# smellslikeml/distributed-deep-learning-workshop

Hardware: AMD Instinct MI355X
Metric: images/sec (whole node) ResNet-50 224px (higher is better)
Workload: dtype bf16; 1 GPU; model=resnet50, global_batch=256, per_gpu_batch=256, image_size=224, parallelism=dp1, hip_ops=True, conv_routes=hip

## Files before the change

ddlw_amd/ops/abi.py:

```python
from __future__ import annotations

import ctypes
from ctypes import POINTER, c_char_p, c_float, c_int, c_long, c_ulonglong


class Ptr(ctypes.c_void_p):

    @classmethod
    def from_param(cls, v):
        if v is None or isinstance(v, int):
            return ctypes.c_void_p(v)
        return ctypes.c_void_p(v.data_ptr())


def long_array(values):
    return (c_long * len(values))(*values)


def int_array(values):
    return (c_int * len(values))(*values)


_P, _I, _L, _F = Ptr, c_int, c_long, c_float

SIGNATURES = {
    "ddlw_last_error": (c_char_p, []),
    "ddlw_device_sync": (_I, []),
    "ddlw_bn_nparts": (_I, [_L, _I]),
    "ddlw_bn_stats": (_I, [_P, _P, _P, _L, _I, _P]),
    "ddlw_bn_parts_fold": (_I, [_P, _P, _P, _P, _L, _I, _I, _P]),
    "ddlw_bn_finalize": (_I, [_P] * 6 + [_L, _I, _I, _F, _F, _P]),
    "ddlw_bn_apply": (_I, [_P] * 8 + [_L, _I, _I, _P]),
    "ddlw_bn_bwd_reduce": (_I, [_P] * 7 + [_L, _I, _I, _P]),
    "ddlw_bn_grad_finalize": (_I, [_P, _P, _P, _P, _I, _I, _P]),
    "ddlw_bn_bwd_dx": (_I, [_P] * 10 + [_L, _I, _I, _P]),
    "ddlw_maxpool3x3s2_fwd": (_I, [_P, _P, _P] + [_I] * 6 + [_P]),
    "ddlw_maxpool3x3s2_bwd": (_I, [_P, _P, _P] + [_I] * 6 + [_P]),
    "ddlw_gap_fwd": (_I, [_P, _P, _I, _I, _I, _P]),
    "ddlw_gap_bwd": (_I, [_P, _P, _I, _I, _I, _P]),
    "ddlw_softmax_ce": (_I, [_P, _P, _P, _P, _I, _I, _F, _P]),
    "ddlw_dropout_fwd": (_I, [_P, _P, _P, _L, _F, c_ulonglong, _P]),
    "ddlw_dropout_bwd": (_I, [_P, _P, _P, _L, _F, _P]),
    "ddlw_argmax_rows": (_I, [_P, _P, _L, _I, _P]),
    "ddlw_accuracy": (_I, [_P, _P, _P, _L, _I, _P]),
    "ddlw_ce_metrics_nblocks": (_I, [_I, _I, _P]),
    "ddlw_ce_metrics": (_I, [_P] * 6 + [_I, _I, _F, _I, _P]),
    "ddlw_normalize_u8": (_I, [_P, _P, _L, _P]),
    "ddlw_fused_sgd": (_I, [_P, _I, _L, _F, _F, _F, _I, _P]),
    "ddlw_fused_adam": (_I, [_P, _I, _L, _F, _F, _F, _F, _F, _F, _F, _P]),
    "ddlw_fused_adadelta": (_I, [_P, _I, _L, _F, _F, _F, _F, _P]),
    "ddlw_depthwise_fwd": (_I, [_P, _P, _P] + [_I] * 10 + [_P]),
    "ddlw_depthwise_fwd_ep": (_I, [_P] * 5 + [_I] * 9 + [_P]),
    "ddlw_depthwise_dgrad": (_I, [_P, _P, _P] + [_I] * 10 + [_P]),
    "ddlw_depthwise_wgrad_nparts": (_I, [_L, _I]),
    "ddlw_depthwise_wgrad": (_I, [_P, _P, _P, _P] + [_I] * 10 + [_P]),
    "ddlw_pw_conv_fwd": (_I, [_P] * 6 + [_I, _L, _I, _I, _P]),
    "ddlw_pw_conv_nparts": (_I, [_L, _I, _P]),
    "ddlw_pw_conv_fwd_stats": (_I, [_P] * 5 + [_L, _I, _I, _P]),
    "ddlw_conv_fwd_nparts": (_L, [_I] * 8),
    "ddlw_conv_fwd_igemm": (_I, [_P] * 14 + [_I] * 15 + [_P]),
    "ddlw_conv_dgrad_s2m": (_I, [_P] * 4 + [_I] * 9
                            + [POINTER(c_long), POINTER(c_long), POINTER(c_int), _P]),
    "ddlw_conv_wgrad": (_I, [_P] * 5 + [_I] * 12 + [_P]),
    "ddlw_stem_repack": (_I, [_P, _P, _I, _I, _I, _P]),
    "ddlw_conv_stem": (_I, [_P] * 4 + [_I] * 8 + [_P, _P, _I, _P]),
    "ddlw_stem_wgrad": (_I, [_P] * 5 + [_I] * 7 + [_P]),
    "ddlw_stem3_u8_fwd_ep": (_I, [_P] * 5 + [_I] * 6 + [_P]),
}


def apply(cdll, on_missing) -> None:
    for name, (restype, argtypes) in SIGNATURES.items():
        try:
            fn = getattr(cdll, name)
        except AttributeError:
            on_missing(name)
            raise
        fn.restype = restype
        fn.argtypes = argtypes
```

ddlw_amd/ops/conv_gemm.py:

```python
from __future__ import annotations

import json
import os
from pathlib import Path
from typing import Tuple

import torch

from .abi import int_array, long_array
from .runtime import launch, query

_DISPATCH_PATH = Path(__file__).resolve().parent / "conv_dispatch.json"
_dispatch = None


def _table() -> dict:
    global _dispatch
    if _dispatch is None:
        if _DISPATCH_PATH.exists():
            _dispatch = json.loads(_DISPATCH_PATH.read_text())
        else:
            _dispatch = {}
    return _dispatch


def _key(N, H, W, C, K, R, S, stride) -> str:
    return f"{N}x{H}x{W}x{C}-{K}k{R}x{S}s{stride}"


def fwd_supported(C: int, K: int, R: int, S: int) -> bool:
    return C % 64 == 0


def dgrad_supported(C: int, K: int, stride, R: int = 1, pad: int = 0) -> bool:
    s = stride[0] if isinstance(stride, (tuple, list)) else stride
    if K % 64 != 0:
        return False
    if s == 1:
        return True
    return s == 2 and ((R == 1 and pad == 0) or (R == 3 and pad == 1))


_zpage = {}


def _zero_page(device) -> torch.Tensor:
    t = _zpage.get(device)
    if t is None:
        t = torch.zeros(64, dtype=torch.bfloat16, device=device)
        _zpage[device] = t
    return t


def _route(kind: str, shape_key: str, mode: str, supported: bool) -> bool:
    if not supported:
        return False
    if mode == "hip":
        return True
    if mode == "stock":
        return False
    ent = _table().get(shape_key)
    if ent is None:
        return False
    return ent.get(kind, "stock") == "hip"


def _pair(v) -> Tuple[int, int]:
    return (v, v) if isinstance(v, int) else (int(v[0]), int(v[1]))


def _igemm(x, w, y, N, H, W, C, K, Ho, Wo, R, S, stride, pad, oH, oW, oS,
           acc=None, parts=None, bnb=(None,) * 4, ep=(None, None, 0),
           acc_mask=None):
    ps, pq = (None, None) if parts is None else (parts[0], parts[1])
    launch("conv_fwd_igemm", x, w, y, _zero_page(x.device), acc, acc_mask,
           ps, pq, *bnb,
           ep[0], ep[1], 1 if ep[2] else 0,
           N, H, W, C, K, Ho, Wo, R, S, stride, pad, oH, oW, oS)


def conv_fwd_kernel(x: torch.Tensor, weight: torch.Tensor, stride, padding,
                    acc: torch.Tensor = None, bn_parts: bool = False,
                    bnb=None, ep=None, acc_mask: torch.Tensor = None):
    n, c, h, w = x.shape
    k, _, r, s = weight.shape
    st, _ = _pair(stride)
    pd, _ = _pair(padding)
    ho = (h + 2 * pd - r) // st + 1
    wo = (w + 2 * pd - s) // st + 1
    x = x.contiguous(memory_format=torch.channels_last)
    weight = weight.contiguous(memory_format=torch.channels_last)
    y = torch.empty((n, k, ho, wo), dtype=torch.bfloat16, device=x.device,
                    memory_format=torch.channels_last)
    if acc is not None:
        assert acc.shape == y.shape and acc.dtype == torch.bfloat16
        acc = acc.contiguous(memory_format=torch.channels_last)
    if acc_mask is not None and acc is not None:
        assert (acc_mask.dtype == torch.uint8 and acc_mask.is_contiguous()
                and acc_mask.numel() * 8 == y.numel())
    bnb_args, ep_args = (None,) * 4, (None, None, 0)
    parts = np_ = None
    if ep is not None:
        ep_args = ep
    elif bnb is not None or bn_parts:
        if bnb is not None:
            bx, bmask, bmean, brstd = bnb
            bx = bx.contiguous(memory_format=torch.channels_last)
            bnb_args = (bx, bmask, bmean, brstd)
        else:
            assert acc is None
        np_ = int(query("conv_fwd_nparts", n, c, k, ho, wo, r, s,
                        1 if bnb is not None else 0))
        parts = torch.empty(2, np_, k, dtype=torch.float32, device=x.device)
    _igemm(x, weight, y, n, h, w, c, k, ho, wo, r, s, st, pd, ho, wo, 1,
           acc, parts, bnb_args, ep_args, acc_mask)
    return y if parts is None else (y, parts, np_)


def wgrad_supported(C: int, K: int) -> bool:
    return C % 8 == 0 and K % 8 == 0


def _wgrad_split(M: int, K: int, C: int, RS: int) -> int:
    bk = 128 if K >= 128 else 64
    bc = 128 if C >= 128 else 64
    base = ((K + bk - 1) // bk) * ((C + bc - 1) // bc) * RS
    split = max(1, min(1024 // max(base, 1), 1024, M // 64 or 1))
    return split


def conv_wgrad_kernel(dy: torch.Tensor, x: torch.Tensor, weight_shape,
                      stride, padding) -> torch.Tensor:
    n, c, h, w = x.shape
    k, _, r, s = weight_shape
    st, _ = _pair(stride)
    pd, _ = _pair(padding)
    ho, wo = dy.shape[2], dy.shape[3]
    M = n * ho * wo
    split = _wgrad_split(M, k, c, r * s)
    x = x.contiguous(memory_format=torch.channels_last)
    dy = dy.contiguous(memory_format=torch.channels_last)
    elems = k * r * s * c
    slab = torch.empty(split * elems, dtype=torch.float32, device=x.device)
    dw = torch.empty((k, c, r, s), dtype=torch.bfloat16, device=x.device,
                     memory_format=torch.channels_last)
    launch("conv_wgrad", dy, x, _zero_page(x.device), slab, dw,
           n, h, w, c, k, ho, wo, r, s, st, pd, split)
    return dw


def conv_dgrad_kernel(dy: torch.Tensor, weight: torch.Tensor, in_shape,
                      padding, stride=1, acc: torch.Tensor = None, bnb=None,
                      acc_mask: torch.Tensor = None):
    k, c, r, s = weight.shape
    pd, _ = _pair(padding)
    st, _ = _pair(stride)
    wt = weight.flip(2, 3).permute(1, 0, 2, 3)
    wt = wt.contiguous(memory_format=torch.channels_last)
    if st == 1:
        return conv_fwd_kernel(dy, wt, 1, r - 1 - pd, acc=acc, bnb=bnb,
                               acc_mask=acc_mask)
    assert acc is None and acc_mask is None, \
        "fused accumulate: stride-1 dgrad only"
    assert bnb is None, "fused BN-bwd reduce: stride-1 dgrad only"
    if st == 2 and r == 3 and pd == 1:
        return _conv_dgrad_s2_3x3(dy, weight, in_shape)
    assert st == 2 and r == 1 and pd == 0, "scatter dgrad: 1x1 s2 pad0 only"
    n, _, ho, wo = dy.shape
    _, _, ih, iw = in_shape
    dy = dy.contiguous(memory_format=torch.channels_last)
    dx = torch.empty((n, c, ih, iw), dtype=torch.bfloat16, device=dy.device,
                     memory_format=torch.channels_last).zero_()
    _igemm(dy, wt, dx, n, ho, wo, k, c, ho, wo, 1, 1, 1, 0, ih, iw, 2)
    return dx


def _raw_fwd_scatter(x, wflat, y_ptr, N, H, W, C, K, Ho, Wo, R, S,
                     oH, oW, oS):
    _igemm(x, wflat, y_ptr, N, H, W, C, K, Ho, Wo, R, S, 1, 0, oH, oW, oS)


def _conv_dgrad_s2_3x3(dy: torch.Tensor, weight: torch.Tensor, in_shape) -> torch.Tensor:
    k, c, _, _ = weight.shape
    n, _, ih, iw = in_shape
    ho, wo = dy.shape[2], dy.shape[3]
    dy = dy.contiguous(memory_format=torch.channels_last)
    dx = torch.empty((n, c, ih, iw), dtype=torch.bfloat16, device=dy.device,
                     memory_format=torch.channels_last)
    classes = []
    for dh in (0, 1):
        taps_r = [r for r in (2, 1, 0) if (dh + 1 - r) % 2 == 0]
        for dw_ in (0, 1):
            taps_s = [t for t in (2, 1, 0) if (dw_ + 1 - t) % 2 == 0]
            sub = weight[:, :, taps_r][:, :, :, taps_s]
            wf = sub.permute(1, 0, 2, 3).contiguous(
                memory_format=torch.channels_last)
            classes.append((dh, dw_, len(taps_r), len(taps_s),
                            (dh * iw + dw_) * c, wf))
    if ih % 2 == 0 and iw % 2 == 0 and k % 64 == 0:
        wcat = torch.cat([wf.permute(0, 2, 3, 1).reshape(-1)
                          for *_, wf in classes])
        woffs = [0]
        for *_, wf in classes[:-1]:
            woffs.append(woffs[-1] + wf.numel())
        launch("conv_dgrad_s2m", dy, wcat, dx, _zero_page(dy.device),
               n, ho, wo, k, c, ih // 2, iw // 2, ih, iw,
               long_array(woffs),
               long_array([off for _, _, _, _, off, _ in classes]),
               int_array([v for _, _, nr, ns, _, _ in classes for v in (nr, ns)]))
        return dx
    for dh, dw_, nr, ns, off_elems, wf in classes:
        oh = (ih - dh + 1) // 2
        ow = (iw - dw_ + 1) // 2
        _raw_fwd_scatter(
            dy, wf, dx.data_ptr() + off_elems * dx.element_size(),
            n, ho, wo, k, c, oh, ow, nr, ns, ih, iw, 2,
        )
    return dx


def conv_backward(dy, x, weight, stride, padding, hip_dgrad, hip_wgrad,
                  need_dx=True, need_dw=True, acc=None, acc_mask=None):
    if acc_mask is not None and not (need_dx and hip_dgrad
                                     and _pair(stride)[0] == 1):
        raise ValueError("conv_backward: acc_mask needs the stride-1 HIP dgrad")
    dy = dy.contiguous(memory_format=torch.channels_last)
    if dy.is_cuda and dy.dtype != torch.bfloat16:
        dy = dy.to(torch.bfloat16)
    st, _ = _pair(stride)
    dx = dw = None
    if need_dx and hip_dgrad:
        fuse = acc if st == 1 else None
        dx = conv_dgrad_kernel(dy, weight.to(torch.bfloat16), x.shape,
                               padding, stride, acc=fuse, acc_mask=acc_mask)
        if acc is not None and fuse is None:
            dx = dx + acc
    if need_dw and hip_wgrad:
        dw = conv_wgrad_kernel(dy, x, weight.shape, stride, padding)
        if dw.dtype != weight.dtype:
            dw = dw.to(weight.dtype)
    if (need_dw and dw is None) or (need_dx and dx is None):
        mask_dx = bool(need_dx and dx is None)
        mask_dw = bool(need_dw and dw is None)
        w16 = weight.to(dy.dtype)
        gi, gw, _ = torch.ops.aten.convolution_backward(
            dy, x, w16, None,
            list(stride) if isinstance(stride, (tuple, list)) else [stride] * 2,
            list(padding) if isinstance(padding, (tuple, list)) else [padding] * 2,
            [1, 1], False, [0, 0], 1,
            [mask_dx, mask_dw, False],
        )
        if mask_dx:
            dx = gi if acc is None else gi + acc
        if mask_dw:
            dw = gw.to(weight.dtype)
    return dx, dw


class _ConvFn(torch.autograd.Function):
    @staticmethod
    def forward(ctx, x, weight, bias, stride, padding, hip_fwd, hip_dgrad,
                hip_wgrad):
        ctx.save_for_backward(x, weight)
        ctx.stride, ctx.padding = stride, padding
        ctx.hip_dgrad = hip_dgrad
        ctx.hip_wgrad = hip_wgrad
        ctx.has_bias = bias is not None
        if hip_fwd:
            y = conv_fwd_kernel(x, weight.to(torch.bfloat16), stride, padding)
        else:
            y = torch.nn.functional.conv2d(
                x, weight.to(x.dtype), None, stride, padding
            )
        if bias is not None:
            y = y + bias.to(y.dtype).view(1, -1, 1, 1)
        return y

    @staticmethod
    def backward(ctx, dy):
        x, weight = ctx.saved_tensors
        dx, dw = conv_backward(
            dy, x, weight, ctx.stride, ctx.padding,
            ctx.hip_dgrad, ctx.hip_wgrad,
            need_dx=ctx.needs_input_grad[0], need_dw=ctx.needs_input_grad[1],
        )
        db = None
        if ctx.has_bias and ctx.needs_input_grad[2]:
            db = dy.float().sum(dim=(0, 2, 3))
        return dx, dw, db, None, None, None, None, None


def available(mod, x: torch.Tensor, mode: str) -> bool:
    if mode == "stock":
        return False
    cache = getattr(mod, "_ddlw_cache", None)
    sig = (tuple(x.shape), mode)
    if cache is not None and cache[0] == sig:
        mod._ddlw_route = cache[1]
        return cache[1][0] or cache[1][1]
    n, c, h, w = x.shape
    k, _, r, s = mod.weight.shape
    st, _ = _pair(mod.stride)
    key = _key(n, h, w, c, k, r, s, st)
    pd0 = mod.padding[0] if isinstance(mod.padding, (tuple, list)) else mod.padding
    f = _route("fwd", key, mode, fwd_supported(c, k, r, s))
    d = _route("dgrad", key, mode, dgrad_supported(c, k, mod.stride, r, pd0))
    g = _route("wgrad", key, mode, wgrad_supported(c, k))
    mod._ddlw_route = (f, d, g)
    mod._ddlw_cache = (sig, (f, d, g))
    return f or d or g


def conv2d(x, weight, bias, stride, padding, hip_fwd: bool, hip_dgrad: bool,
           hip_wgrad: bool = False):
    return _ConvFn.apply(x, weight, bias, stride, padding, hip_fwd, hip_dgrad,
                         hip_wgrad)




def _stem_repack(x: torch.Tensor) -> torch.Tensor:
    n, _, h, w = x.shape
    x4 = torch.empty((n, h, w + 8, 4), dtype=torch.bfloat16, device=x.device)
    launch("stem_repack", x, x4, n, h, w)
    return x4


def stem_fwd_kernel(x: torch.Tensor, weight: torch.Tensor,
                    ep=None) -> torch.Tensor:
    n, c, h, w = x.shape
    k = weight.shape[0]
    assert c == 3 and k == 64 and weight.shape[2:] == (7, 7)
    ho, wo = (h + 6 - 7) // 2 + 1, (w + 6 - 7) // 2 + 1
    x = x.contiguous(memory_format=torch.channels_last)
    dev = x.device
    x4 = _stem_repack(x)
    w4 = torch.zeros(k, 8, 8, 4, dtype=torch.bfloat16, device=dev)
    w4[:, :7, :7, :3] = weight.detach().to(torch.bfloat16).permute(0, 2, 3, 1)
    y = torch.empty((n, k, ho, wo), dtype=torch.bfloat16, device=dev,
                    memory_format=torch.channels_last)
    es, eb, relu = ep if ep is not None else (None, None, False)
    launch("conv_stem", x4, w4, y, _zero_page(dev), n, h, w, k, ho, wo, 2, 3,
           es, eb, 1 if relu else 0)
    return y


def stem_wgrad_kernel(dy: torch.Tensor, x: torch.Tensor) -> torch.Tensor:
    n, c, h, w = x.shape
    assert c == 3
    ho, wo = dy.shape[2], dy.shape[3]
    x = x.contiguous(memory_format=torch.channels_last)
    dy = dy.contiguous(memory_format=torch.channels_last)
    dev = x.device
    x4 = _stem_repack(x)
    split = int(min(1024, max(1, (n * ho * wo) // 64)))
    slab = torch.empty(split * 64 * 256, dtype=torch.float32, device=dev)
    dw4 = torch.empty(64, 256, dtype=torch.bfloat16, device=dev)
    launch("stem_wgrad", dy, x4, _zero_page(dev), slab, dw4,
           n, h, w, 64, ho, wo, split)
    dw = (dw4.view(64, 8, 8, 4)[:, :7, :7, :3]
          .permute(0, 3, 1, 2)
          .contiguous(memory_format=torch.channels_last))
    return dw


class _StemFn(torch.autograd.Function):
    @staticmethod
    def forward(ctx, x, weight):
        ctx.save_for_backward(x, weight)
        return stem_fwd_kernel(x, weight)

    @staticmethod
    def backward(ctx, dy):
        x, weight = ctx.saved_tensors
        dy = dy.contiguous(memory_format=torch.channels_last)
        dx = dw = None
        if ctx.needs_input_grad[0]:
            dx = torch.nn.grad.conv2d_input(
                list(x.shape), weight.to(dy.dtype), dy, (2, 2), (3, 3))
        if ctx.needs_input_grad[1]:
            if dy.is_cuda and dy.dtype == torch.bfloat16:
                dw = stem_wgrad_kernel(dy, x).to(weight.dtype)
            else:
                dw = torch.nn.grad.conv2d_weight(
                    x.to(dy.dtype), list(weight.shape), dy, (2, 2), (3, 3))
        return dx, dw


def stem_conv2d(x: torch.Tensor, weight: torch.Tensor) -> torch.Tensor:
    return _StemFn.apply(x, weight)
```

ddlw_amd/ops/hip/conv_wgrad.hip:

```cpp
#include "igemm.h"

typedef __attribute__((ext_vector_type(8))) __bf16 bf16x8_v;
typedef __attribute__((ext_vector_type(4))) float f32x4_v;
typedef __attribute__((ext_vector_type(2))) unsigned tr64_t;

__device__ __forceinline__ unsigned lds_u32(const bf16_t* p) {
  return (unsigned)(unsigned long long)(const LDS_AS bf16_t*)p;
}

template <int BK, int BC, int WG_BM = 64>
__global__ __launch_bounds__(256) void k_conv_wgrad(
    const bf16_t* __restrict__ dy, const bf16_t* __restrict__ x,
    const bf16_t* __restrict__ zpage,
    float* __restrict__ slab,
    int N, int H, int W_, int C, int K, int Ho, int Wo,
    int R, int S, int stride, int pad,
    int split, long m_per_split,
    unsigned long long magic_wo, unsigned shift_wo,
    unsigned long long magic_ho, unsigned shift_ho) {
  constexpr int WK = BK / 2, WC = BC / 2;
  constexpr int KF = WK / 16, CF = WC / 16;
  constexpr int MG = WG_BM / 32;
  constexpr int PA = BK / 16 * MG;
  constexpr int PB = BC / 16 * MG;
  constexpr int TILE = WG_BM * BK;
  constexpr int BUF = WG_BM * (BK + BC);
  __shared__ __attribute__((aligned(16))) bf16_t smem[2 * BUF];

  const long M = (long)N * Ho * Wo;
  const int ctiles = (C + BC - 1) / BC;
  const int tile_k = blockIdx.x / ctiles;
  const int tile_c = blockIdx.x % ctiles;
  const int rs = blockIdx.y;
  const int r = rs / S, s = rs % S;
  const int sp = blockIdx.z;

  const long m0 = (long)sp * m_per_split;
  const long m1 = (m0 + m_per_split < M) ? (m0 + m_per_split) : M;

  const int tid = threadIdx.x;
  const int lane = tid & 63;
  const int wave = tid >> 6;
  const int wr = wave >> 1, wc2 = wave & 1;

  const int s_pos = lane >> 3;
  const int s_mr = (lane >> 1) & 3;
  const int s_half = lane & 1;
  const int s_mb = (s_pos < 4) ? (2 * s_pos) : (2 * (s_pos - 4) + 1);
  const int s_mlocal = s_mb * 4 + s_mr;
  const int s_koff = s_half * 8;

  const bf16_t* dyrow[MG];
  const bf16_t* xrow[MG];
  bool dv[MG], xv[MG];

  auto decompose = [&](long mbase) {
    #pragma unroll
    for (int g = 0; g < MG; ++g) {
      long m = mbase + g * 32 + s_mlocal;
      dv[g] = m < m1;
      dyrow[g] = dv[g] ? (dy + m * K) : zpage;
      bool ok = false;
      const bf16_t* xr = zpage;
      if (m < m1) {
        unsigned mu = (unsigned)m;
        unsigned q1 = mdiv(mu, magic_wo, shift_wo);
        int wo = (int)(mu - q1 * (unsigned)Wo);
        unsigned n_u = mdiv(q1, magic_ho, shift_ho);
        int ho = (int)(q1 - n_u * (unsigned)Ho);
        int hh = ho * stride - pad + r;
        int wwv = wo * stride - pad + s;
        ok = hh >= 0 && hh < H && wwv >= 0 && wwv < W_;
        if (ok) xr = x + (((long)(int)n_u * H + hh) * W_ + wwv) * C;
      }
      xv[g] = ok;
      xrow[g] = xr;
    }
  };

  auto stage = [&](int buf) {
    bf16_t* ldy = smem + buf * BUF;
    bf16_t* lx = ldy + TILE;
    #pragma unroll
    for (int p = wave; p < PA; p += 4) {
      const int k16 = p / MG, g = p % MG;
      int kk = tile_k * BK + k16 * 16 + s_koff;
      const bf16_t* src = (dv[g] && kk < K) ? (dyrow[g] + kk) : zpage;
      __builtin_amdgcn_global_load_lds(
          (const GLOBAL_AS void*)src, (LDS_AS void*)(ldy + p * 512), 16, 0, 0);
    }
    #pragma unroll
    for (int p = wave; p < PB; p += 4) {
      const int c16 = p / MG, g = p % MG;
      int cc = tile_c * BC + c16 * 16 + s_koff;
      const bf16_t* src = (xv[g] && cc < C) ? (xrow[g] + cc) : zpage;
      __builtin_amdgcn_global_load_lds(
          (const GLOBAL_AS void*)src, (LDS_AS void*)(lx + p * 512), 16, 0, 0);
    }
  };

  f32x4_v acc[KF][CF];
  #pragma unroll
  for (int a = 0; a < KF; ++a)
    #pragma unroll
    for (int b = 0; b < CF; ++b) acc[a][b] = {0.f, 0.f, 0.f, 0.f};

  const long nsteps = (m1 - m0 + WG_BM - 1) / WG_BM;
  decompose(m0);
  stage(0);
  if (1 < nsteps) decompose(m0 + WG_BM);
  __syncthreads();

  int cur = 0;
  for (long t = 0; t < nsteps; ++t) {
    if (t + 1 < nsteps) {
      stage(cur ^ 1);
      if (t + 2 < nsteps) decompose(m0 + (t + 2) * WG_BM);
    }
    bf16_t* ldy = smem + cur * BUF;
    bf16_t* lx = ldy + TILE;
    #pragma unroll
    for (int mh = 0; mh < MG; ++mh) {
      tr64_t fk0[KF], fk1[KF], fc0[CF], fc1[CF];
      #pragma unroll
      for (int a = 0; a < KF; ++a) {
        const int k16 = (wr * WK) / 16 + a;
        unsigned addr = lds_u32(ldy + ((k16 * MG + mh) * 8) * 64) + lane * 8;
        asm volatile("ds_read_b64_tr_b16 %0, %1" : "=v"(fk0[a]) : "v"(addr));
        asm volatile("ds_read_b64_tr_b16 %0, %1 offset:512"
                     : "=v"(fk1[a]) : "v"(addr));
      }
      #pragma unroll
      for (int b = 0; b < CF; ++b) {
        const int c16 = (wc2 * WC) / 16 + b;
        unsigned addr = lds_u32(lx + ((c16 * MG + mh) * 8) * 64) + lane * 8;
        asm volatile("ds_read_b64_tr_b16 %0, %1" : "=v"(fc0[b]) : "v"(addr));
        asm volatile("ds_read_b64_tr_b16 %0, %1 offset:512"
                     : "=v"(fc1[b]) : "v"(addr));
      }
      asm volatile("s_waitcnt lgkmcnt(0)" ::: "memory");
      __builtin_amdgcn_sched_barrier(0);
      #pragma unroll
      for (int a = 0; a < KF; ++a)
        #pragma unroll
        for (int b = 0; b < CF; ++b) {
          union { struct { tr64_t lo, hi; } p; bf16x8_v v; } fa, fb;
          fa.p.lo = fk0[a]; fa.p.hi = fk1[a];
          fb.p.lo = fc0[b]; fb.p.hi = fc1[b];
          acc[a][b] = __builtin_amdgcn_mfma_f32_16x16x32_bf16(
              fa.v, fb.v, acc[a][b], 0, 0, 0);
        }
    }
    __syncthreads();
    cur ^= 1;
  }

  const long RSC = (long)R * S * C;
  float* out = slab + (long)sp * K * RSC;
  const int d_c = lane & 15;
  const int d_k0 = (lane >> 4) * 4;
  #pragma unroll
  for (int a = 0; a < KF; ++a) {
    #pragma unroll
    for (int b = 0; b < CF; ++b) {
      int c = tile_c * BC + wc2 * WC + b * 16 + d_c;
      if (c >= C) continue;
      #pragma unroll
      for (int q = 0; q < 4; ++q) {
        int k = tile_k * BK + wr * WK + a * 16 + d_k0 + q;
        if (k < K) out[(long)k * RSC + (long)rs * C + c] = acc[a][b][q];
      }
    }
  }
}

__global__ __launch_bounds__(256) void k_wgrad_reduce(
    const float* __restrict__ slab, bf16_t* __restrict__ dw,
    long elems, int split) {
  const int el = threadIdx.x & 31;
  const int pg = threadIdx.x >> 5;
  __shared__ float lds[8][32];
  for (long i0 = (long)blockIdx.x * 32; i0 < elems; i0 += (long)gridDim.x * 32) {
    const long i = i0 + el;
    float a = 0.f;
    if (i < elems)
      for (int p = pg; p < split; p += 8) a += slab[(long)p * elems + i];
    lds[pg][el] = a;
    __syncthreads();
    if (pg == 0 && i < elems) {
      #pragma unroll
      for (int g = 1; g < 8; ++g) a += lds[g][el];
      union { float f; unsigned u; } cvt;
      cvt.f = a;
      unsigned rb = 0x7FFF + ((cvt.u >> 16) & 1);
      dw[i] = (bf16_t)((cvt.u + rb) >> 16);
    }
    __syncthreads();
  }
}

DDLW_EXPORT int ddlw_conv_wgrad(const void* dy, const void* x, const void* zpage,
                                void* slab, void* dw, int N, int H, int W_,
                                int C, int K, int Ho, int Wo, int R, int S,
                                int stride, int pad, int split, void* stream) {
  if (C % 8 != 0 || K % 8 != 0) {
    ddlw_set_error("conv_wgrad: C and K must be multiples of 8");
    return 2;
  }
  long M = (long)N * Ho * Wo;
  if (M >= (1ll << 31)) {
    ddlw_set_error("conv_wgrad: M >= 2^31 unsupported");
    return 2;
  }
  unsigned long long mg_wo, mg_ho;
  unsigned sh_wo, sh_ho;
  make_magic((unsigned)Wo, &mg_wo, &sh_wo);
  make_magic((unsigned)Ho, &mg_ho, &sh_ho);
  long m_per_split = cdiv(M, split);
  hipStream_t st = (hipStream_t)stream;
#define WLAUNCH3(BK, BC, BM_)                                                 \
  do {                                                                        \
    dim3 grid((int)(cdiv(K, BK) * cdiv(C, BC)), R * S, split);                \
    hipLaunchKernelGGL((k_conv_wgrad<BK, BC, BM_>), grid, dim3(256), 0, st,   \
                       (const bf16_t*)dy, (const bf16_t*)x,                   \
                       (const bf16_t*)zpage, (float*)slab, N, H, W_, C, K,    \
                       Ho, Wo, R, S, stride, pad, split, m_per_split, mg_wo,  \
                       sh_wo, mg_ho, sh_ho);                                  \
  } while (0)
#define WLAUNCH(BK, BC)                                                       \
  do {                                                                        \
    dim3 grid((int)(cdiv(K, BK) * cdiv(C, BC)), R * S, split);                \
    hipLaunchKernelGGL((k_conv_wgrad<BK, BC>), grid, dim3(256), 0, st,        \
                       (const bf16_t*)dy, (const bf16_t*)x,                   \
                       (const bf16_t*)zpage, (float*)slab, N, H, W_, C, K,    \
                       Ho, Wo, R, S, stride, pad, split, m_per_split, mg_wo,  \
                       sh_wo, mg_ho, sh_ho);                                  \
  } while (0)
  if (K >= 128 && C >= 128) WLAUNCH(128, 128);
  else if (C >= 128) WLAUNCH(64, 128);
  else if (K >= 128) WLAUNCH(128, 64);
  else WLAUNCH(64, 64);
#undef WLAUNCH
#undef WLAUNCH3
  {
    hipError_t err_ = hipGetLastError();
    if (err_ != hipSuccess) { ddlw_set_error(hipGetErrorString(err_)); return 1; }
  }
  long elems = (long)K * R * S * C;
  long g = cdiv(elems, 32);
  if (g > 4096) g = 4096;
  hipLaunchKernelGGL(k_wgrad_reduce, dim3((int)g), dim3(256), 0, st,
                     (const float*)slab, (bf16_t*)dw, elems, split);
  DDLW_CHECK_LAUNCH();
}
```

Baseline: 8876 images/sec.

## Add fused 9-tap wgrad kernel for 3x3 stride-1 convolutions

Adds a dedicated weight-gradient kernel for 3x3 stride-1 pad-1 convolutions. Each block stages a ring of input rows and dy rows in LDS and accumulates all nine taps from one dy fragment load, so input and dy are reused across taps instead of being re-read by per-tap GEMMs. Routing defaults to padded widths 32 and 64, which covers the ResNet-50 3x3 layers at 56 and 28 spatial width. The cost is heavy register use for nine accumulator sets, which may lower occupancy, plus a new split heuristic.

```diff
diff --git a/ddlw_amd/ops/abi.py b/ddlw_amd/ops/abi.py
--- a/ddlw_amd/ops/abi.py
+++ b/ddlw_amd/ops/abi.py
@@ -62,6 +62,7 @@
     "ddlw_conv_dgrad_s2m": (_I, [_P] * 4 + [_I] * 9
                             + [POINTER(c_long), POINTER(c_long), POINTER(c_int), _P]),
     "ddlw_conv_wgrad": (_I, [_P] * 5 + [_I] * 12 + [_P]),
+    "ddlw_conv_wgrad3x3": (_I, [_P] * 5 + [_I] * 10 + [_P]),
     "ddlw_stem_repack": (_I, [_P, _P, _I, _I, _I, _P]),
     "ddlw_conv_stem": (_I, [_P] * 4 + [_I] * 8 + [_P, _P, _I, _P]),
     "ddlw_stem_wgrad": (_I, [_P] * 5 + [_I] * 7 + [_P]),
diff --git a/ddlw_amd/ops/conv_gemm.py b/ddlw_amd/ops/conv_gemm.py
--- a/ddlw_amd/ops/conv_gemm.py
+++ b/ddlw_amd/ops/conv_gemm.py
@@ -129,8 +129,77 @@
     return split
 
 
+def wgrad3x3_supported(C: int, K: int, R: int, S: int, stride: int,
+                       pad: int, W: int) -> bool:
+    return (R == 3 and S == 3 and stride == 1 and pad == 1
+            and C % 64 == 0 and K % 64 == 0 and 1 <= W <= 64)
+
+
+def _padded_width(W: int) -> int:
+    return 8 if W <= 8 else 16 if W <= 16 else 32 if W <= 32 else 64
+
+
+_TAPS_DEFAULT_PW = frozenset({64, 32})
+
+
+def wgrad3x3_routed(C, K, R, S, stride, pad, W) -> bool:
+    lever = os.environ.get("DDLW_WGRAD_TAPS", "")
+    if lever == "0" or not wgrad3x3_supported(C, K, R, S, stride, pad, W):
+        return False
+    return lever == "1" or _padded_width(W) in _TAPS_DEFAULT_PW
+
+
+def wgrad3x3_slices(rows: int, split: int):
+    split = max(1, min(int(split), rows))
+    q, rem = divmod(rows, split)
+    out, start = [], 0
+    for i in range(split):
+        end = start + q + (1 if i < rem else 0)
+        out.append((start, end))
+        start = end
+    return out
+
+
+def _wgrad3x3_split(rows: int, K: int, C: int, W: int) -> int:
+    tiles = max(1, (K // 64) * (C // 64))
+    target = 256 if W > 32 else 512
+    return max(1, min(target // tiles, rows, 65535))
+
+
+def conv_wgrad3x3_kernel(dy: torch.Tensor, x: torch.Tensor, weight_shape,
+                         stride=1, padding=1, split: int = None) -> torch.Tensor:
+    n, c, h, w = x.shape
+    k, _, r, s = weight_shape
+    st, _ = _pair(stride)
+    pd, _ = _pair(padding)
+    rows = n * h
+    if split is None:
+        split = _wgrad3x3_split(rows, k, c, w)
+    split = max(1, min(int(split), rows))
+    x = x.contiguous(memory_format=torch.channels_last)
+    dy = dy.contiguous(memory_format=torch.channels_last)
+    slab = torch.empty(split * k * r * s * c, dtype=torch.float32,
+                       device=x.device)
+    dw = torch.empty((k, c, r, s), dtype=torch.bfloat16, device=x.device,
+                     memory_format=torch.channels_last)
+    launch("conv_wgrad3x3", dy, x, _zero_page(x.device), slab, dw,
+           n, h, w, c, k, r, s, st, pd, split)
+    return dw
+
+
 def conv_wgrad_kernel(dy: torch.Tensor, x: torch.Tensor, weight_shape,
                       stride, padding) -> torch.Tensor:
+    n, c, h, w = x.shape
+    k, _, r, s = weight_shape
+    st, _ = _pair(stride)
+    pd, _ = _pair(padding)
+    if wgrad3x3_routed(c, k, r, s, st, pd, w):
+        return conv_wgrad3x3_kernel(dy, x, weight_shape, st, pd)
+    return conv_wgrad_pertap_kernel(dy, x, weight_shape, st, pd)
+
+
+def conv_wgrad_pertap_kernel(dy: torch.Tensor, x: torch.Tensor, weight_shape,
+                             stride, padding) -> torch.Tensor:
     n, c, h, w = x.shape
     k, _, r, s = weight_shape
     st, _ = _pair(stride)
diff --git a/ddlw_amd/ops/hip/conv_wgrad.hip b/ddlw_amd/ops/hip/conv_wgrad.hip
--- a/ddlw_amd/ops/hip/conv_wgrad.hip
+++ b/ddlw_amd/ops/hip/conv_wgrad.hip
@@ -253,3 +253,240 @@
                      (const float*)slab, (bf16_t*)dw, elems, split);
   DDLW_CHECK_LAUNCH();
 }
+
+template <int PW>
+__global__ __launch_bounds__(256) void k_conv_wgrad3x3(
+    const bf16_t* __restrict__ dy, const bf16_t* __restrict__ x,
+    const bf16_t* __restrict__ zpage,
+    float* __restrict__ slab,
+    int N, int H, int W_, int C, int K,
+    int rows_q, int rows_rem,
+    unsigned long long magic_h, unsigned shift_h) {
+  constexpr int RPS = PW >= 32 ? 1 : 32 / PW;
+  constexpr int SM = RPS * PW;
+  constexpr int MG = SM / 32;
+  constexpr int NR = 4 * RPS;
+  constexpr int BPR = PW / 4;
+  constexpr int EB = BPR < 8 ? BPR : 8;
+  constexpr int PP = PW / 8;
+  constexpr int ROWIMG = PW * 64;
+  constexpr int SLOT = 3 * ROWIMG + (PW == 8 ? 64 : 0);
+  constexpr int DYIMG = SM * 64;
+  constexpr unsigned ODD = EB / 2 * 128;
+  __shared__ __attribute__((aligned(16))) bf16_t smem[2 * DYIMG + NR * SLOT];
+  bf16_t* const xring = smem + 2 * DYIMG;
+
+  const int ctiles = C / 64;
+  const int tile_k = blockIdx.x / ctiles;
+  const int tile_c = blockIdx.x % ctiles;
+  const int sp = blockIdx.y;
+  const int tid = threadIdx.x;
+  const int lane = tid & 63;
+  const int wave = __builtin_amdgcn_readfirstlane(tid >> 6);
+  const int wr = wave >> 1, wc2 = wave & 1;
+
+  const int g0 = sp * rows_q + (sp < rows_rem ? sp : rows_rem);
+  const int gl = g0 + rows_q + (sp < rows_rem ? 1 : 0) - 1;
+  const int n0 = (int)mdiv((unsigned)g0, magic_h, shift_h);
+  const int n1 = (int)mdiv((unsigned)gl, magic_h, shift_h);
+  const int ho0 = g0 - n0 * H;
+  const int L = (n1 - n0) * (H + 1) + (gl - n1 * H) - ho0 + 1;
+  const int nsteps = (L + RPS - 1) / RPS;
+
+  const int s_pos = lane >> 3;
+  const int s_mr = (lane >> 1) & 3;
+  const int s_koff = (lane & 1) * 8;
+
+  int xn = n0, xhp = ho0, xrel = 0;
+  int dn = n0, dhp = ho0 + 1, drel = 1;
+
+  auto stage_x = [&](auto count) {
+    constexpr int COUNT = decltype(count)::value;
+    constexpr int TOTAL = COUNT * 3 * PP;
+    #pragma unroll
+    for (int i = 0; i < (TOTAL + 3) / 4; ++i) {
+      const int idx = i * 4 + wave;
+      if (TOTAL % 4 != 0 && idx >= TOTAL) break;
+      const int ric = idx / (3 * PP);
+      const int s = (idx / PP) % 3;
+      const int p = idx % PP;
+      int n = xn, hp = xhp + ric;
+      while (hp > H) { hp -= H + 1; ++n; }
+      const int rel = xrel + ric;
+      const bool rowok = hp >= 1 && rel <= L + 1 && n < N;
+      const int P = p * 8 + s_pos;
+      const int c16 = P / BPR;
+      const int e = P % EB;
+      const int b = e < EB / 2 ? 2 * e : 2 * (e - EB / 2) + 1;
+      const int wo = ((P % BPR) / EB * EB + b) * 4 + s_mr;
+      const int w = wo + s - 1;
+      const bool ok = rowok && wo < W_ && w >= 0 && w < W_;
+      const bf16_t* src =
+          ok ? x + (((long)n * H + (hp - 1)) * W_ + w) * C + tile_c * 64 +
+                   c16 * 16 + s_koff
+             : zpage;
+      bf16_t* dst = xring + (rel & (NR - 1)) * SLOT + s * ROWIMG + p * 512;
+      __builtin_amdgcn_global_load_lds((const GLOBAL_AS void*)src,
+                                       (LDS_AS void*)dst, 16, 0, 0);
+    }
+    xhp += COUNT;
+    while (xhp > H) { xhp -= H + 1; ++xn; }
+    xrel += COUNT;
+  };
+
+  auto stage_dy = [&](int buf) {
+    bf16_t* ldy = smem + buf * DYIMG;
+    #pragma unroll
+    for (int i = 0; i < MG; ++i) {
+      const int idx = i * 4 + wave;
+      const int k16 = idx / MG, g = idx % MG;
+      const int b = s_pos < 4 ? 2 * s_pos : 2 * (s_pos - 4) + 1;
+      const int ms = g * 32 + b * 4 + s_mr;
+      const int ri = ms / PW, wo = ms % PW;
+      int n = dn, hp = dhp + ri;
+      while (hp > H) { hp -= H + 1; ++n; }
+      const bool ok = hp >= 1 && drel + ri <= L && wo < W_;
+      const bf16_t* src =
+          ok ? dy + (((long)n * H + (hp - 1)) * W_ + wo) * K + tile_k * 64 +
+                   k16 * 16 + s_koff
+             : zpage;
+      __builtin_amdgcn_global_load_lds((const GLOBAL_AS void*)src,
+                                       (LDS_AS void*)(ldy + idx * 512), 16, 0, 0);
+    }
+    dhp += RPS;
+    while (dhp > H) { dhp -= H + 1; ++dn; }
+    drel += RPS;
+  };
+
+  f32x4_v acc[9][2][2];
+  #pragma unroll
+  for (int t9 = 0; t9 < 9; ++t9)
+    #pragma unroll
+    for (int a = 0; a < 2; ++a)
+      #pragma unroll
+      for (int b = 0; b < 2; ++b) acc[t9][a][b] = {0.f, 0.f, 0.f, 0.f};
+
+  const int f_q = lane >> 4;
+  const int f_ri = (f_q * 8) / PW;
+  const int f_blk = ((f_q * 8) % PW) / 8;
+  const unsigned f_x = lds_u32(xring) + (unsigned)(wc2 * 2 * BPR + f_blk) * 128 +
+                       (lane & 15) * 8;
+  const unsigned f_dy = lds_u32(smem) + (unsigned)(wr * 2 * MG) * 1024 + lane * 8;
+
+  stage_x(std::integral_constant<int, 2>{});
+  stage_x(std::integral_constant<int, RPS>{});
+  stage_dy(0);
+  __syncthreads();
+
+  int cur = 0;
+  for (int t = 0; t < nsteps; ++t) {
+    if (t + 1 < nsteps) {
+      stage_dy(cur ^ 1);
+      stage_x(std::integral_constant<int, RPS>{});
+    }
+    unsigned xa[3];
+    #pragma unroll
+    for (int r = 0; r < 3; ++r)
+      xa[r] = f_x + (unsigned)((t * RPS + f_ri + r) & (NR - 1)) * (SLOT * 2);
+    const unsigned da = f_dy + (unsigned)cur * (DYIMG * 2);
+    #pragma unroll
+    for (int g = 0; g < MG; ++g) {
+      tr64_t fk[2][2], fx[2][2][2];
+      #pragma unroll
+      for (int a = 0; a < 2; ++a) {
+        const unsigned addr = da + (a * MG + g) * 1024;
+        asm volatile("ds_read_b64_tr_b16 %0, %1" : "=v"(fk[a][0]) : "v"(addr));
+        asm volatile("ds_read_b64_tr_b16 %0, %1 offset:512"
+                     : "=v"(fk[a][1]) : "v"(addr));
+      }
+      auto load_tap = [&](int tap, int fb) {
+        const int r = tap / 3, s = tap % 3;
+        #pragma unroll
+        for (int b = 0; b < 2; ++b) {
+          const unsigned addr =
+              xa[r] + (unsigned)(s * ROWIMG * 2 + b * BPR * 128 + g * 1024);
+          asm volatile("ds_read_b64_tr_b16 %0, %1"
+                       : "=v"(fx[fb][b][0]) : "v"(addr));
+          asm volatile("ds_read_b64_tr_b16 %0, %1"
+                       : "=v"(fx[fb][b][1]) : "v"(addr + ODD));
+        }
+      };
+      load_tap(0, 0);
+      #pragma unroll
+      for (int tap = 0; tap < 9; ++tap) {
+        asm volatile("s_waitcnt lgkmcnt(0)" ::: "memory");
+        __builtin_amdgcn_sched_barrier(0);
+        if (tap + 1 < 9) load_tap(tap + 1, (tap + 1) & 1);
+        #pragma unroll
+        for (int a = 0; a < 2; ++a)
+          #pragma unroll
+          for (int b = 0; b < 2; ++b) {
+            union { struct { tr64_t lo, hi; } p; bf16x8_v v; } fa, fb;
+            fa.p.lo = fk[a][0]; fa.p.hi = fk[a][1];
+            fb.p.lo = fx[tap & 1][b][0]; fb.p.hi = fx[tap & 1][b][1];
+            acc[tap][a][b] = __builtin_amdgcn_mfma_f32_16x16x32_bf16(
+                fa.v, fb.v, acc[tap][a][b], 0, 0, 0);
+          }
+      }
+    }
+    __syncthreads();
+    cur ^= 1;
+  }
+
+  const long RSC = 9l * C;
+  float* out = slab + (long)sp * K * RSC;
+  const int c0 = tile_c * 64 + wc2 * 32 + (lane & 15);
+  const int k0 = tile_k * 64 + wr * 32 + (lane >> 4) * 4;
+  #pragma unroll
+  for (int tap = 0; tap < 9; ++tap)
+    #pragma unroll
+    for (int a = 0; a < 2; ++a)
+      #pragma unroll
+      for (int b = 0; b < 2; ++b)
+        #pragma unroll
+        for (int q = 0; q < 4; ++q)
+          out[(long)(k0 + a * 16 + q) * RSC + tap * C + c0 + b * 16] =
+              acc[tap][a][b][q];
+}
+
+DDLW_EXPORT int ddlw_conv_wgrad3x3(const void* dy, const void* x,
+                                   const void* zpage, void* slab, void* dw,
+                                   int N, int H, int W_, int C, int K, int R,
+                                   int S, int stride, int pad, int split,
+                                   void* stream) {
+  const char* who = "conv_wgrad3x3";
+  if (R != 3 || S != 3) return ddlw_fail(who, "R and S must be 3");
+  if (stride != 1) return ddlw_fail(who, "stride must be 1");
+  if (pad != 1) return ddlw_fail(who, "pad must be 1");
+  if (C % 64 != 0 || K % 64 != 0)
+    return ddlw_fail(who, "C and K must be multiples of 64");
+  if (N < 1 || H < 1 || W_ < 1 || W_ > 64)
+    return ddlw_fail(who, "width must be 1..64");
+  const long rows = (long)N * H;
+  if ((long)N * (H + 1) * W_ >= (1ll << 31))
+    return ddlw_fail(who, "N*(H+1)*W >= 2^31 unsupported");
+  if (split < 1 || split > rows || split > 65535)
+    return ddlw_fail(who, "split must be 1..min(N*H, 65535)");
+  unsigned long long mg_h;
+  unsigned sh_h;
+  make_magic((unsigned)H, &mg_h, &sh_h);
+  hipStream_t st = (hipStream_t)stream;
+  dim3 grid((K / 64) * (C / 64), split);
+  const int pw = W_ <= 8 ? 8 : W_ <= 16 ? 16 : W_ <= 32 ? 32 : 64;
+  with_int<8, 16, 32, 64>(pw, [&](auto PWc) {
+    hipLaunchKernelGGL((k_conv_wgrad3x3<decltype(PWc)::value>), grid,
+                       dim3(256), 0, st, (const bf16_t*)dy, (const bf16_t*)x,
+                       (const bf16_t*)zpage, (float*)slab, N, H, W_, C, K,
+                       (int)(rows / split), (int)(rows % split), mg_h, sh_h);
+  });
+  {
+    hipError_t err_ = hipGetLastError();
+    if (err_ != hipSuccess) { ddlw_set_error(hipGetErrorString(err_)); return 1; }
+  }
+  long elems = (long)K * 9 * C;
+  long g = cdiv(elems, 32);
+  if (g > 4096) g = 4096;
+  hipLaunchKernelGGL(k_wgrad_reduce, dim3((int)g), dim3(256), 0, st,
+                     (const float*)slab, (bf16_t*)dw, elems, split);
+  DDLW_CHECK_LAUNCH();
+}
```

Measured after the change: 8999 images/sec, median of 6. 1.4% higher.
